# p1an-lin-jung/WavThruVec_pytorch

Measured on AMD Instinct MI355X. Metric: audio samples/sec (16 kHz) Vec2Wav generator, B=32×256-frame 768-d latents, 1/2/4/8 GPU, higher is better.
Workload: dtype f32; 1 GPU; BASELINE configs[1]: B=32/GPU x T=256 frames, 768-d latents, upsample (5,4,4,2,2) x320, ResBlock2, train-mode CondBN, f32; global_batch=32, frames=256, parallelism=single GPU

## Files before the change

### include/vec2wav_hip.h

```cpp
#ifndef VEC2WAV_HIP_H
#define VEC2WAV_HIP_H

#include <stdint.h>

#ifdef __cplusplus
extern "C" {
#endif

#define V2W_ABI_VERSION 35

#define V2W_E_ARG      (-1)
#define V2W_E_SHAPE    (-2)
#define V2W_E_ALGO     (-3)

#define V2W_ALGO_AUTO   0
#define V2W_ALGO_DIRECT 1
#define V2W_ALGO_MFMA   2
#define V2W_ALGO_BF16   4
#define V2W_ALGO_SPLIT  3
#define V2W_ALGO_WINO   5

int         v2w_abi_version(void);
const char* v2w_build_arch(void);

typedef struct { uint64_t magic; char* buf; int32_t cap; int32_t len; } v2w_name_sink;
#define V2W_NAME_SINK_MAGIC 0x5632574e414d4531ull
#define V2W_NAME_SINK_STREAM(sink) ((void*)((uintptr_t)(sink) | (uintptr_t)1))

int v2w_wn_fold_conv (const float* v, const float* g, float* wf, float* scratch,
                      int c_out, int c_in, int k, void* stream);
int v2w_wn_fold_convt(const float* v, const float* g, float* wf, float* scratch,
                      int c_in, int c_out, int k, void* stream);

int v2w_wf_transpose_flip(const float* wf, float* out, int k, int c_in, int c_out, void* stream);
int v2w_wf_gather_transpose(const float* wf, float* out, int k, int c_in, int c_out, int t_start, int t_step, int n, void* stream);

int v2w_pack_mfma(const float* wf, float* wp, int k, int c_in, int c_out, int u, void* stream);
int v2w_pack_mfma_dgrad(const float* wf, float* wp, int k, int c_in, int c_out, void* stream);
int v2w_pack_mfma_batch(const float* wf, float* wp, int k, int c_in, int c_out, int u, int n, void* stream);
int v2w_pack_wino(const float* wf, float* wpw, int k, int c_in, int c_out, void* stream);
int v2w_wino_terms(int k);

typedef struct {
    const float* v; const float* g; float* wp; float* scale;
    int32_t c_in, c_out, k, u, transposed;
    int32_t mf, ck;
    int32_t _pad;
    float* wf;
    float* wpd;
    float* wpw;
} v2w_fold_desc;
int v2w_fold_plan(v2w_fold_desc* descs, int n, int32_t* starts);
int v2w_fold_pack_batch(const v2w_fold_desc* descs_dev, const int32_t* starts_dev, int n,
                        int nblk_scale, int nblk_pack, int lds_bytes, void* stream);

typedef struct {
    const float* in;   const float* in_a;  const float* in_s;
    const float* wf;
    const float* wp;
    const float* bias;
    const float* res;  const float* res_a; const float* res_s;
    const float* add0; const float* add1;
    const float* mask_src; const float* mask_a; const float* mask_s;
    float*       out;
    int32_t B, C_in, C_out, L, k, dil;
    float   slope;
    int32_t accumulate;
    float   out_div;
    int32_t algo;
    float   mask_slope;
    int32_t in_stride, in_phase;
    int32_t pad_left;
    const void*  wps;
    const float* winv;
    int32_t in_ct, out_ct;
    float   out_slope;
    int32_t io_bf16;
    float*  rowsum_part;
    float*  splitk_ws;
    int64_t splitk_ws_bytes;
// ... 365 lines not shown
```

### wavthruvec_pytorch_amd/_hip.py

```python
from __future__ import annotations

import ctypes as C
import os
import threading

from . import build as _build

ABI_VERSION = 35
V2W_MAX_STAGES = 8
V2W_BN_SPLITS = 64
ALGO_AUTO, ALGO_DIRECT, ALGO_MFMA, ALGO_SPLIT, ALGO_BF16, ALGO_WINO = 0, 1, 2, 3, 4, 5

_fp = C.c_void_p


class Conv1dArgs(C.Structure):
    _fields_ = [('in_', _fp), ('in_a', _fp), ('in_s', _fp), ('wf', _fp), ('wp', _fp), ('bias', _fp),
                ('res', _fp), ('res_a', _fp), ('res_s', _fp), ('add0', _fp), ('add1', _fp),
                ('mask_src', _fp), ('mask_a', _fp), ('mask_s', _fp), ('out', _fp),
                ('B', C.c_int32), ('C_in', C.c_int32), ('C_out', C.c_int32), ('L', C.c_int32),
                ('k', C.c_int32), ('dil', C.c_int32), ('slope', C.c_float), ('accumulate', C.c_int32),
                ('out_div', C.c_float), ('algo', C.c_int32), ('mask_slope', C.c_float),
                ('in_stride', C.c_int32), ('in_phase', C.c_int32), ('pad_left', C.c_int32),
                ('wps', _fp), ('winv', _fp), ('in_ct', C.c_int32), ('out_ct', C.c_int32), ('out_slope', C.c_float),
                ('io_bf16', C.c_int32), ('rowsum_part', _fp), ('splitk_ws', _fp), ('splitk_ws_bytes', C.c_int64)]


class ConvT1dArgs(C.Structure):
    _fields_ = [('in_', _fp), ('wf', _fp), ('wp', _fp), ('bias', _fp), ('out', _fp), ('stats_part', _fp),
                ('B', C.c_int32), ('C_in', C.c_int32), ('C_out', C.c_int32), ('L', C.c_int32),
                ('k', C.c_int32), ('u', C.c_int32), ('slope', C.c_float), ('algo', C.c_int32), ('io_bf16', C.c_int32), ('_pad', C.c_int32),
                ('splitk_ws', _fp), ('splitk_ws_bytes', C.c_int64)]


class PairArgs(C.Structure):
    _fields_ = [('in_', _fp), ('in_a', _fp), ('in_s', _fp), ('wp1', _fp), ('bias1', _fp), ('wp2', _fp), ('bias2', _fp),
                ('add0', _fp), ('add1', _fp), ('out', _fp),
                ('B', C.c_int32), ('C', C.c_int32), ('L', C.c_int32), ('k', C.c_int32), ('dil1', C.c_int32), ('dil2', C.c_int32),
                ('res_mode', C.c_int32), ('slope', C.c_float), ('out_div', C.c_float)]


class StageArgs(C.Structure):
    _fields_ = [('in_', _fp), ('in_a', _fp), ('in_s', _fp),
                ('wp1', _fp * 4), ('bias1', _fp * 4), ('wp2', _fp * 4), ('bias2', _fp * 4),
                ('k', C.c_int32 * 4), ('dil1', C.c_int32 * 4), ('dil2', C.c_int32 * 4),
                ('out', _fp), ('nk', C.c_int32), ('B', C.c_int32), ('C', C.c_int32), ('L', C.c_int32),
                ('slope', C.c_float), ('out_div', C.c_float),
                ('post_w', _fp), ('post_b', _fp), ('post_out', _fp), ('post_k', C.c_int32), ('post_slope', C.c_float),
                ('bwd_mask1', _fp * 4), ('bwd_mid', _fp * 4), ('bwd_mask2', _fp), ('bwd_mask2_a', _fp), ('bwd_mask2_s', _fp),
                ('bwd_slope', C.c_float), ('bwd_rowsum', _fp * 4)]


class FoldDesc(C.Structure):
    _fields_ = [('v', _fp), ('g', _fp), ('wp', _fp), ('scale', _fp),
                ('c_in', C.c_int32), ('c_out', C.c_int32), ('k', C.c_int32), ('u', C.c_int32), ('transposed', C.c_int32),
                ('mf', C.c_int32), ('ck', C.c_int32), ('_pad', C.c_int32), ('wf', _fp), ('wpd', _fp), ('wpw', _fp)]


_P4 = _fp * 4
_I4 = C.c_int32 * 4


class StageSplitArgs(C.Structure):
    _fields_ = [('in_', _fp), ('in_a', _fp), ('in_s', _fp),
                ('wps1', _P4), ('sc1', _P4), ('bias1', _P4), ('wps2', _P4), ('sc2', _P4), ('bias2', _P4),
                ('k', _I4), ('dil1', _I4), ('dil2', _I4), ('out', _fp),
                ('nk', C.c_int32), ('B', C.c_int32), ('C', C.c_int32), ('L', C.c_int32),
                ('slope', C.c_float), ('out_div', C.c_float), ('bf16', C.c_int32), ('io_bf16', C.c_int32),
                ('post_w', _fp), ('post_b', _fp), ('post_out', _fp), ('post_k', C.c_int32), ('post_slope', C.c_float),
                ('up_wps', _fp), ('up_bias', _fp), ('up_out', _fp), ('up_stats_part', _fp),
                ('up_k', C.c_int32), ('up_u', C.c_int32), ('up_slope', C.c_float), ('rb1', C.c_int32),
                ('in_b', _P4), ('out_b', _P4), ('add0', _fp), ('add1', _fp)]


class BranchConvsArgs(C.Structure):
    _fields_ = [('in_', _fp * 3), ('in_a', _fp), ('in_s', _fp), ('wps', _fp * 3), ('bias', _fp * 3), ('out', _fp * 3),
                ('k', C.c_int32 * 3), ('dil', C.c_int32 * 3),
                ('nbr', C.c_int32), ('mode', C.c_int32), ('B', C.c_int32), ('C', C.c_int32), ('L', C.c_int32),
                ('slope', C.c_float), ('out_div', C.c_float), ('_pad', C.c_int32)]


class SplitDesc(C.Structure):
    _fields_ = [('v', _fp), ('g', _fp), ('wps', _fp), ('sc', _fp), ('rowscale', _fp),
                ('c_in', C.c_int32), ('c_out', C.c_int32), ('k', C.c_int32), ('mode', C.c_int32)]


_PA = _fp * V2W_MAX_STAGES


# ... 332 lines not shown
```

### wavthruvec_pytorch_amd/csrc/v2w_conv_mfma.hip

```cpp
#include <type_traits>
#include "v2w_tile.h"
#include "v2w_internal.h"
#include "v2w_wino.h"

#ifdef V2W_TIMELINE
V2W_TL_SETTER(v2w_timeline_set_tile)
#endif

namespace {

template <int MF, int U, int MI, int NI, int WM, int WN, int CK, int NPF, int RING, int EPI, bool VEC>
__global__ void __launch_bounds__(64 * WM * WN, (U == 1 && MI * NI >= 4) ? 3 : 1)
conv_tile_kernel(const MultiArgs m) {
    constexpr bool LEN = EPI == 3;
    typedef Frag<MF> F;
    typedef typename F::acc_t acc_t;
    constexpr int NTHREADS = 64 * WM * WN;
    constexpr int MT = MF * MI * WM;
    constexpr int NT = MF * NI * WN;
    constexpr int KSTEP = F::KSTEP;
    constexpr int CKG = 4 * KSTEP;
    constexpr int GPC = CK / CKG;
    constexpr int RS = TileGeom<MF, CK>::RS;
    static_assert(CK % CKG == 0, "chunk must hold whole A fragments");
    static_assert(RING == 2 || (RING == 4 && GPC == 4), "the 4-deep ring walks exactly one tap per revolution");

    extern __shared__ __attribute__((aligned(16))) float smem[];

    int pq = 0;
#pragma unroll
    for (int i = 1; i < V2W_MAX_MULTI; ++i) pq += (int)blockIdx.x >= m.start[i] ? 1 : 0;
    const TileArgs& p = m.p[pq];
    const int mtiles = p.Cout / MT;
// ... 665 lines not shown
                const int t0 = (r + pad) % U, nt = (K - t0 + U - 1) / U;
                if (left < nt) { t = t0 + left * U; break; }
                left -= nt;
            }
        }
        const int c = ch * CK + gg * CKG + j * KSTEP + lane / MF;
        const int co = mb * MF + lane % MF;
        wp[o] = tflip ? wf[((size_t)(K - 1 - t) * Cout + co) * Cin + c] : wf[((size_t)t * Cin + c) * Cout + co];
    }
}


__device__ __forceinline__ int find_layer(const int32_t* __restrict__ starts, int n, int blk) {
    int lo = 0, hi = n;
    while (hi - lo > 1) { const int mid = (lo + hi) >> 1; if (starts[mid] <= blk) lo = mid; else hi = mid; }
    return lo;
}

__global__ void __launch_bounds__(256)
fold_scale_batch_kernel(const v2w_fold_desc* __restrict__ descs, const int32_t* __restrict__ starts, int n) {
    __shared__ double red[16];
    const int li = find_layer(starts, n, blockIdx.x);
    const v2w_fold_desc d = descs[li];
    const int row = blockIdx.x - starts[li];
    const int inner = (d.transposed ? d.c_out : d.c_in) * d.k;
    const float* src = d.v + (size_t)row * inner;
    double acc = 0.0;
    if (d.g)
        for (int i = threadIdx.x; i < inner; i += 256) { const double x = (double)src[i]; acc += x * x; }
    const double n2 = v2w_block_sum(acc, red);
    if (threadIdx.x == 0) d.scale[row] = d.g ? (float)((double)d.g[row] / sqrt(n2)) : 1.f;
}

__global__ void __launch_bounds__(256)
fold_pack_batch_kernel(const v2w_fold_desc* __restrict__ descs, const int32_t* __restrict__ starts, int n) {
    extern __shared__ float tile[];
    const int li = find_layer(starts, n, blockIdx.x);
    const v2w_fold_desc d = descs[li];
    const int blk = blockIdx.x - starts[li];
    const int MF = d.mf, CK = d.ck, K = d.k, U = d.u;
    const int KSTEP = MF == 32 ? 2 : 4, CKG = 4 * KSTEP, GPC = CK / CKG, nch = d.c_in / CK;
    const int mb = blk / nch, ch = blk % nch;
    const int nrow = d.transposed ? CK : MF;
    const int rlen = (d.transposed ? MF : CK) * K;
    const int rstride = rlen + 1;
    for (int idx = threadIdx.x; idx < nrow * rlen; idx += 256) {
        const int r = idx / rlen, x = idx - r * rlen;
        const float* src = d.transposed ? d.v + ((size_t)(ch * CK + r) * d.c_out + mb * MF) * K
                                        : d.v + ((size_t)(mb * MF + r) * d.c_in + ch * CK) * K;
        const float sc = d.scale[d.transposed ? ch * CK + r : mb * MF + r];
        tile[r * rstride + x] = src[x] * sc;
    }
    __syncthreads();
    const int pad = (K - U) / 2;
    float* dst = d.wp + (size_t)(mb * nch + ch) * K * GPC * 256;
    for (int o = threadIdx.x; o < K * GPC * 256; o += 256) {
        const int j = o & 3, lane = (o >> 2) & 63;
        const int rest = o >> 8;
        const int gg = rest % GPC, ts = rest / GPC;
        int t = ts;
        if (U > 1) {
            int left = ts;
            for (int r = 0; r < U; ++r) {
                const int t0 = (r + pad) % U, nt = (K - t0 + U - 1) / U;
                if (left < nt) { t = t0 + left * U; break; }
                left -= nt;
            }
        }
        const int c = gg * CKG + j * KSTEP + lane / MF, co = lane % MF;
        dst[o] = d.transposed ? tile[c * rstride + co * K + t] : tile[co * rstride + c * K + t];
    }
    if (d.wpw && d.transposed) {
        constexpr int NT = wino_seg_terms(2), WGPC = 4;
        const int nchw = nch / 2;
        for (int o = threadIdx.x; o < U * GPC * NT * 256; o += 256) {
            const int j = o & 3, lane = (o >> 2) & 63;
            int rest = o >> 8;
            const int term = rest % NT; rest /= NT;
            const int g2 = rest % GPC, r = rest / GPC;
            const int row = r * 32 + lane % 32, co = row / U, ph = row - co * U;
            const int c = g2 * CKG + j * KSTEP + lane / MF;
            const float* w = tile + c * rstride + co * K;
            const int fi = ((ch & 1) * GPC + g2) * NT + term;
            d.wpw[((((size_t)(mb * U + r) * nchw + ch / 2) * (NT * WGPC) + fi) * 64 + lane) * 4 + j] = wino_weight(2, term, w[ph + U], w[ph], 0.f);
        }
    } else if (d.wpw) {
        const int nfr = wino_terms(K) * GPC;
        float* dw = d.wpw + (size_t)(mb * nch + ch) * nfr * 256;
        for (int o = threadIdx.x; o < nfr * 256; o += 256) {
            const int j = o & 3, lane = (o >> 2) & 63;
            int s0, ntap, gg, term;
            wino_frag(K, GPC, o >> 8, s0, ntap, gg, term);
            const int c = gg * CKG + j * KSTEP + lane / MF, co = lane % MF;
            const float* w = tile + co * rstride + c * K + s0;
            dw[o] = wino_weight(ntap, term, w[0], ntap > 1 ? w[1] : 0.f, ntap > 2 ? w[2] : 0.f);
        }
    }
    if (d.wf) {
        for (int idx = threadIdx.x; idx < K * CK * MF; idx += 256) {
            const int col = idx % MF, c = (idx / MF) % CK, t = idx / (MF * CK);
            d.wf[((size_t)t * d.c_in + ch * CK + c) * d.c_out + mb * MF + col] =
                d.transposed ? tile[c * rstride + col * K + t] : tile[col * rstride + c * K + t];
        }
    }
    if (d.wpd) {
        const int nchd = d.c_out / CK;
        float* dd = d.wpd + (size_t)(ch * nchd + mb) * K * GPC * 256;
        for (int o = threadIdx.x; o < K * GPC * 256; o += 256) {
            const int j = o & 3, lane = (o >> 2) & 63;
            const int rest = o >> 8;
            const int gg = rest % GPC, ts = rest / GPC;
            const int kc = gg * CKG + j * KSTEP + lane / MF, row = lane % MF;
            dd[o] = tile[kc * rstride + row * K + (K - 1 - ts)];
        }
    }
}

}

struct LayerCfg { int mf, ck; };
static LayerCfg v2w_layer_cfg(int c_in, int c_out, int u) {
    LayerCfg c{0, 0};
    if (c_in % 16 != 0) return c;
    if (u == 1) {
        if (c_out % 32 == 0 && c_in % 32 == 0) c = {32, 32};
        else if (c_out % 32 == 0) c = {32, 16};
        else if (c_out == 16) c = {16, 16};
    } else if (u == 2 || u == 4 || u == 5 || u == 8) {
        if (c_out % 64 == 0 || c_out == 32) c = {32, 16};
        else if (c_out == 16) c = {16, 16};
    }
    return c;
}

static int pack_mfma(const float* wf, float* wp, int k, int c_in, int c_out, int u, int n, int tflip, void* stream) {
    if (!wf || !wp || k <= 0 || c_in <= 0 || c_out <= 0 || u <= 0) return V2W_E_ARG;
    const LayerCfg cfg = v2w_layer_cfg(c_in, c_out, u);
    if (!cfg.mf) return V2W_E_SHAPE;
    const size_t total = (size_t)k * c_in * c_out;
    int grid = (int)((total + 255) / 256); if (grid > 4096) grid = 4096;
    V2W_LAUNCH(pack_mfma_kernel, dim3(grid, n), dim3(256), 0, (hipStream_t)stream, wf, wp, k, c_in, c_out, cfg.mf, cfg.ck, u, tflip);
    return v2w_launch_status();
}

extern "C" int v2w_pack_mfma(const float* wf, float* wp, int k, int c_in, int c_out, int u, void* stream) {
    return pack_mfma(wf, wp, k, c_in, c_out, u, 1, 0, stream);
}

// ... 60 lines not shown
}

int v2w_convt1d_mfma(const v2w_convt1d_args* a, hipStream_t stream, int* cfg_out, long long* ws_query, const int32_t* len, int len_mul) {
    const LayerCfg cfg = v2w_layer_cfg(a->C_in, a->C_out, a->u);
    if ((!a->wp && !cfg_out && !ws_query) || !cfg.mf) return V2W_E_SHAPE;
    TileArgs p{};
    p.cfg_out = cfg_out;
    p.splitk_ws = a->splitk_ws; p.splitk_ws_bytes = a->splitk_ws ? a->splitk_ws_bytes : 0; p.ws_query = ws_query;
    p.in = a->in; p.wp = a->wp; p.bias = a->bias; p.out = a->out; p.stats_part = a->stats_part;
    if (len && (len_mul < 1 || a->stats_part)) return V2W_E_ARG;
    p.len = len; p.len_mul = len_mul;
    p.B = a->B; p.Cin = a->C_in; p.Cout = a->C_out; p.L = a->L; p.K = a->k; p.dil = 1;
    p.CinT = p.Cin; p.CoutT = p.Cout; p.out_slope = 1.f;
    p.pad = (a->k - a->u) / 2;
    p.slope = a->slope; p.accumulate = 0; p.out_div = 0.f;
    int hl = 0, hr = 0;
    for (int r = 0; r < a->u; ++r) {
        const int rp = r + p.pad, t0 = rp % a->u, c = rp / a->u, nt = (a->k - t0 + a->u - 1) / a->u;
        if (c > hr) hr = c;
        if (nt - 1 - c > hl) hl = nt - 1 - c;
    }
    p.hl = hl; p.hr = hr;
    switch (a->u) {
        case 2: return launch_convt_u<2>(p, stream);
        case 4: return launch_convt_u<4>(p, stream);
        case 5: return launch_convt_u<5>(p, stream);
        case 8: return launch_convt_u<8>(p, stream);
        default: return V2W_E_SHAPE;
    }
}

extern "C" int v2w_fold_plan(v2w_fold_desc* descs, int n, int32_t* starts) {
    if (!descs || !starts || n <= 0) return V2W_E_ARG;
    int bs = 0, bp = 0, lds = 0;
    for (int i = 0; i < n; ++i) {
        v2w_fold_desc& d = descs[i];
        if (d.c_in <= 0 || d.c_out <= 0 || d.k <= 0 || d.u <= 0) return V2W_E_ARG;
        const LayerCfg cfg = v2w_layer_cfg(d.c_in, d.c_out, d.transposed ? d.u : 1);
        if (!cfg.mf) return V2W_E_SHAPE;
        d.mf = cfg.mf; d.ck = cfg.ck;
        if (d.wpd && (d.transposed || d.c_in != d.c_out || cfg.mf != cfg.ck)) return V2W_E_ARG;
        if (d.wpw && !d.transposed && (cfg.mf != 32 || cfg.ck != 32 || wino_terms(d.k) == 0)) return V2W_E_ARG;
        if (d.wpw && d.transposed && (cfg.mf != 32 || cfg.ck != 16 || (d.u != 2 && d.u != 4) || d.k != 2 * d.u || d.c_in % 32 != 0 || d.c_in < 64
                                      || (d.u * d.c_out) % 64 != 0)) return V2W_E_ARG;
        starts[i] = bs; starts[n + 1 + i] = bp;
        bs += d.transposed ? d.c_in : d.c_out;
        bp += (d.c_out / cfg.mf) * (d.c_in / cfg.ck);
        const int nrow = d.transposed ? cfg.ck : cfg.mf, rlen = (d.transposed ? cfg.mf : cfg.ck) * d.k;
        const int bytes = nrow * (rlen + 1) * (int)sizeof(float);
        if (bytes > lds) lds = bytes;
    }
    starts[n] = bs; starts[2 * n + 1] = bp;
    if (lds > 160 * 1024) return V2W_E_SHAPE;
    return lds;
}

extern "C" int v2w_fold_pack_batch(const v2w_fold_desc* descs_dev, const int32_t* starts_dev, int n,
                                   int nblk_scale, int nblk_pack, int lds_bytes, void* stream) {
    if (!descs_dev || !starts_dev || n <= 0 || nblk_scale <= 0 || nblk_pack <= 0 || lds_bytes <= 0) return V2W_E_ARG;
    hipStream_t st = (hipStream_t)stream;
    if (lds_bytes > 64 * 1024) {
        hipError_t e = v2w_max_lds(reinterpret_cast<const void*>(fold_pack_batch_kernel), lds_bytes, st);
        if (e != hipSuccess) return (int)e;
    }
    V2W_LAUNCH(fold_scale_batch_kernel, dim3(nblk_scale), dim3(256), 0, st, descs_dev, starts_dev, n);
    V2W_LAUNCH(fold_pack_batch_kernel, dim3(nblk_pack), dim3(256), lds_bytes, st, descs_dev, starts_dev + n + 1, n);
    return v2w_launch_status();
}
```

### wavthruvec_pytorch_amd/forward_plan.py

```python
from __future__ import annotations

import contextlib
import functools
from collections import namedtuple

import torch

from . import hipops

LRELU_SLOPE = 0.1
POST_SLOPE = 0.01
_Z_CHANNEL = 128


class DirectStreams:

    def __init__(self, main, side, side2=None):
        self.main, self.side, self.side2 = main, side, side if side2 is None else side2
        self.events = {}
        self.nfork = 1
        self.tag = None

    def stream(self, sid):
        return (self.main, self.side, self.side2)[sid]
# ... 192 lines not shown
    @functools.cached_property
    def stg(self):
        return self.g.stage_record(self.stage_i)

    def buf(self, name, shape, dtype=torch.float32):
        return self.g._buf(name, shape, dtype=dtype, device=self.dev)

    def lkw(self, mul=None):
        if self.lens is None:
            return {}
        return dict(lengths=self.lens, len_mul=self.lmul if mul is None else mul)

    def lkw_out(self):
        return self.lkw(self.lmul * self.g.ups[self.stage_i].stride)

    def wino_streams(self, kind='wpw'):
        return self.g._fold_key.get(kind, {})

    def weights(self):
        g, st, dev = self.g, self.st, self.dev
        B, ns = self.B, self.ns
        self.gbs = [self.buf(f'gb.{i}', (B, 2 * g.cbns[i].num_features)) for i in range(ns)]
        self.z_ws = self.buf('z_ws', (ns * B * _Z_CHANNEL,))
        self.sigma_ws = self.buf('sigma_ws', (ns,))
        self.affs = None
        self.cond_ran = False
        if self.cond_sid == 2:
            self.cond()
        with (self.on_side() if st else contextlib.nullcontext()):
            self.wf, self.wp = g._fold_weights(dev, need_wf=self.save is not None, bf16_only=st)
        self.wps = g._split_weights(dev, all_ups=st, ups_stream=self.S.side, mark=self.mark if st else None,
                                    between=self.cond if st else None)
        self.cond()

    def cond(self):
        if self.cond_ran:
            return
        self.cond_ran = True
        g, dev, ns, B = self.g, self.dev, self.ns, self.B
        with self.on_side(self.cond_sid):
            if not self.training and self.save is None:
                sn_p = [q for c in g.cbns for q in (c.layer.weight_orig, c.layer.weight_u, c.layer.weight_v)]
                skey = (tuple((q.data_ptr(), q._version) for q in sn_p), str(dev))
                if g._fold_key.get('sigma') != skey:
                    hipops.cond_sigma([c.layer.weight_orig.detach() for c in g.cbns], [c.layer.weight_u for c in g.cbns],
                                      [c.layer.weight_v for c in g.cbns], self.sigma_ws, training=False)
                    g._fold_key['sigma'] = skey
                self.affs = [(self.buf(f'bn.a{i}', (B, g.cbns[i].num_features)), self.buf(f'bn.s{i}', (B, g.cbns[i].num_features))) for i in range(ns)]
                hipops.cond_affine_eval(
                    self.spk, self.nz, [f.weight.detach() for f in g.fcs], [f.bias.detach() for f in g.fcs],
                    [c.layer.weight_orig.detach() for c in g.cbns], [c.layer.bias.detach() for c in g.cbns], self.sigma_ws,
                    [c.batch_nrom.running_mean for c in g.cbns], [c.batch_nrom.running_var for c in g.cbns],
                    [c.batch_nrom.eps for c in g.cbns], [q[0] for q in self.affs], [q[1] for q in self.affs])
            else:
                g._fold_key.pop('sigma', None)
                hipops.cond_gamma_beta(
                    self.spk, self.nz, [f.weight.detach() for f in g.fcs], [f.bias.detach() for f in g.fcs],
                    [c.layer.weight_orig.detach() for c in g.cbns], [c.layer.bias.detach() for c in g.cbns],
                    [c.layer.weight_u for c in g.cbns], [c.layer.weight_v for c in g.cbns], self.gbs, self.z_ws, self.sigma_ws, self.training)
        if self.st:
            self.mark('cond', self.cond_sid)

    def ck(self, nm, io=3):
        g = self.g
        if nm in self.wps32:
            return dict(algo=hipops.ALGO_BF16, wps=self.wps32[nm])
# ... 388 lines not shown
```

### wavthruvec_pytorch_amd/hipops.py

```python
from __future__ import annotations

import ctypes as C
from typing import Optional, Sequence

import torch

from . import _hip

ALGO_AUTO, ALGO_DIRECT, ALGO_MFMA, ALGO_SPLIT, ALGO_BF16, ALGO_WINO = (_hip.ALGO_AUTO, _hip.ALGO_DIRECT, _hip.ALGO_MFMA, _hip.ALGO_SPLIT,
                                                                        _hip.ALGO_BF16, _hip.ALGO_WINO)


def _chk(t: Optional[torch.Tensor], name: str, dtype=torch.float32):
    if t is None:
        return
    if not t.is_cuda:
        raise RuntimeError(f'{name} must live on a GPU: the Vec2Wav HIP path has no CPU fallback')
    if t.dtype != dtype:
        raise TypeError(f'{name} must be {dtype}, got {t.dtype}')
    if not t.is_contiguous():
        raise RuntimeError(f'{name} must be contiguous')


def _stream(t: torch.Tensor) -> int:
# ... 525 lines not shown


def convt_stats_tiles(B, c_in, c_out, L, k, u):
    cfg = (C.c_int32 * 10)()
    a = _convt_shape(B, c_in, c_out, L, k, u)
    return int(cfg[9]) if _hip.load().v2w_convt1d_tile_config(C.byref(a), cfg) == 0 else 0


def bn_reduce_partials(part, ntiles, Cc, count, stats):
    _hip.check(_hip.load().v2w_bn_reduce_partials(part.data_ptr(), ntiles, Cc, float(count), stats.data_ptr(), _stream(part)),
               'v2w_bn_reduce_partials')
    return stats


def bn_reduce_finalize(part, ntiles, count, stats, gb, running_mean, running_var, num_batches_tracked, a_out, s_out, *, momentum=0.1, eps=1e-5):
    B, C2 = gb.shape
    _hip.check(_hip.load().v2w_bn_reduce_finalize(part.data_ptr(), ntiles, float(count), gb.data_ptr(), running_mean.data_ptr(),
                                                  running_var.data_ptr(), _hip.ptr(num_batches_tracked), stats.data_ptr(), a_out.data_ptr(),
                                                  s_out.data_ptr(), B, C2 // 2, momentum, eps, _stream(gb)), 'v2w_bn_reduce_finalize')
    return a_out, s_out


class FoldPlan:

    def __init__(self, layers, device):
        n = len(layers)
        self.n = n
        layers = [tuple(l) + (None,) * (11 - len(l)) for l in layers]
        rows = [(l[3] if l[7] else l[4]) for l in layers]
        self.scale = torch.empty((sum(rows),), device=device, dtype=torch.float32)
        descs = (_hip.FoldDesc * n)()
        off = 0
        for d, (v, g, wp, ci, co, k, u, tr, wf, wpd, wpw), r in zip(descs, layers, rows):
            d.v = v.data_ptr(); d.g = _hip.ptr(g); d.wp = wp.data_ptr()
            d.wf = _hip.ptr(wf); d.wpd = _hip.ptr(wpd); d.wpw = _hip.ptr(wpw)
            d.scale = self.scale.data_ptr() + 4 * off
            d.c_in, d.c_out, d.k, d.u, d.transposed = ci, co, k, u, int(tr)
            off += r
        starts = (C.c_int32 * (2 * (n + 1)))()
        lds = _hip.load().v2w_fold_plan(descs, n, starts)
        _hip.check(0 if lds > 0 else (lds or -1), 'v2w_fold_plan')
        self.lds = lds
        self.nblk_scale, self.nblk_pack = starts[n], starts[2 * n + 1]
        self.descs_dev = torch.frombuffer(bytearray(bytes(descs)), dtype=torch.uint8).to(device)
        self.starts_dev = torch.tensor(list(starts), dtype=torch.int32, device=device)
        self.key = tuple((v.data_ptr(), 0 if g is None else g.data_ptr(), wp.data_ptr()) for (v, g, wp, *_r) in layers)

    def run(self):
        _hip.check(_hip.load().v2w_fold_pack_batch(self.descs_dev.data_ptr(), self.starts_dev.data_ptr(), self.n,
                                                   self.nblk_scale, self.nblk_pack, self.lds,
                                                   torch.cuda.current_stream(self.scale.device).cuda_stream),
                   'v2w_fold_pack_batch')


class SplitPlan:

    def __init__(self, layers, device, bf16=False):
        n = len(layers)
        self.n = n
        self.bf16 = bool(bf16)
        self.rowscale = torch.empty((sum(v.shape[0] for v, *_ in layers),), device=device, dtype=torch.float32)
        descs = (_hip.SplitDesc * n)()
        starts = [0] * (2 * (n + 1))
        off = blocks = 0
        for i, (d, (v, g, wps, sc)) in enumerate(zip(descs, layers)):
            co, ci, k = v.shape
            d.v = v.data_ptr(); d.g = _hip.ptr(g); d.wps = wps.data_ptr(); d.sc = sc.data_ptr()
            d.rowscale = self.rowscale.data_ptr() + 4 * off
            d.c_in, d.c_out, d.k, d.mode = ci, co, k, int(bf16)
            starts[i], starts[n + 1 + i] = off, blocks
            off += co
            blocks += ((co + 31) // 32) * (ci // 16)
        starts[n], starts[2 * n + 1] = off, blocks
        self.nblk_rows, self.nblk_pack = off, blocks
        self.k_max = max(v.shape[2] for v, *_ in layers)
        self.descs_dev = torch.frombuffer(bytearray(bytes(descs)), dtype=torch.uint8).to(device)
        self.starts_dev = torch.tensor(starts, dtype=torch.int32, device=device)
        self.key = tuple((v.data_ptr(), 0 if g is None else g.data_ptr(), w.data_ptr()) for (v, g, w, _s) in layers)

# ... 894 lines not shown
```

### wavthruvec_pytorch_amd/models.py

```python
from __future__ import annotations

import math
import warnings
from typing import Dict, List, Optional

import contextlib
import torch
import torch.nn as nn

from . import _hip, hipops
from .modules import ConditionalBatchNorm1d
from .utils import get_padding, init_weights

LRELU_SLOPE = 0.1
_SIDE_STREAMS: Dict[str, 'torch.cuda.Stream'] = {}
_CAPTURE_STREAMS: Dict[str, 'torch.cuda.Stream'] = {}
_Z_CHANNEL = 128


class _WNConvBase(nn.Module):
    transposed = False

    def __init__(self, in_channels, out_channels, kernel_size, stride=1, dilation=1, padding=0):
        super().__init__()
# ... 328 lines not shown
        wpw_up = {}
        for name, m in layers:
            if bf16_only and name != 'conv_post':
                wf[name], wp[name] = None, None
                continue
            v, g = (m.weight_v.detach(), m.weight_g.detach()) if m.weight_normed else (m.weight.detach(), None)
            u = m.stride if m.transposed else 1
            mfma_ok = (self.algo != hipops.ALGO_DIRECT and name != 'conv_post' and
                       hipops.conv_tile_config(1, m.in_channels, m.out_channels, 64, m.kernel_size,
                                               1 if m.transposed else m.dilation, u) is not None)
            wpwb = None
            if (mfma_ok and wino and not m.transposed and hipops.wino_terms(m.kernel_size) and m.in_channels % 32 == 0 and m.in_channels >= 64
                    and m.out_channels % 64 == 0 and (m.out_channels >= 128 or m.dilation == 1)):
                wpwb = wpw[name] = self._wbuf('wpw.' + name, (hipops.wino_terms(m.kernel_size) * m.in_channels * m.out_channels,), device=device)
            if mfma_ok and name in stage_names:
                wpwb = wpw_stage[name] = self._wbuf('wpw.' + name, (hipops.wino_terms(m.kernel_size) * m.in_channels * m.out_channels,), device=device)
            if mfma_ok and wpwb is None and name in sum_names:
                wpwb = wpw_sum[name] = self._wbuf('wpw.' + name, (hipops.wino_terms(m.kernel_size) * m.in_channels * m.out_channels,), device=device)
            if mfma_ok and name in up_names:
                wpwb = wpw_up[name] = self._wbuf('wpw.' + name, (3 * m.stride * m.out_channels * m.in_channels,), device=device)
            if mfma_ok and need_wf:
                n_el = m.kernel_size * m.in_channels * m.out_channels
                wfb = self._wbuf('wf.' + name, (m.kernel_size, m.in_channels, m.out_channels), device=device)
                wpb = self._wbuf('wp.' + name, (n_el,), device=device)
                wdb = None
                if not m.transposed and m.in_channels == m.out_channels and name.startswith('resblocks.'):
                    wdb = wpd[name] = self._wbuf('wpd.' + name, (n_el,), device=device)
                batch.append((v, g, wpb, m.in_channels, m.out_channels, m.kernel_size, u, m.transposed, wfb, wdb, wpwb))
                wf[name], wp[name] = wfb, wpb
            elif mfma_ok:
                wpb = self._wbuf('wp.' + name, (m.kernel_size * m.in_channels * m.out_channels,), device=device)
                batch.append((v, g, wpb, m.in_channels, m.out_channels, m.kernel_size, u, m.transposed, None, None, wpwb))
                wf[name], wp[name] = None, wpb
            else:
                wfb = self._wbuf('wf.' + name, (m.kernel_size, m.in_channels, m.out_channels), device=device)
                scratch = self._wbuf('wf_scratch', (max(2048, m.out_channels, m.in_channels),), device=device)
                (hipops.fold_convt_weight if m.transposed else hipops.fold_conv_weight)(v, g, wfb, scratch)
                wf[name], wp[name] = wfb, None
        if batch:
            key = tuple((q[0].data_ptr(), 0 if q[1] is None else q[1].data_ptr(), q[2].data_ptr(),
                         0 if len(q) < 9 or q[8] is None else q[8].data_ptr(), 0 if len(q) < 11 or q[10] is None else q[10].data_ptr()) for q in batch)
            plan = self._fold_key.get('plan')
            if plan is None or plan.key != key:
                self._drop_tapes()
                plan = hipops.FoldPlan(batch, device)
                plan.key = key
                self._fold_key['plan'] = plan
            plan.run()
        self._fold_key.update(state=state, wf=wf, wp=wp, wpd=wpd, wpw=wpw, wpw_stage=wpw_stage, wpw_sum=wpw_sum, wpw_up=wpw_up, vers=tuple(vers), gen=self._fold_key.get('gen', 0) + 1)
        return wf, wp

    def stage_record(self, i):
        from .forward_plan import Stage
        js = range(i * self.num_kernels, (i + 1) * self.num_kernels)
        return Stage(i, self.ups[i].out_channels, tuple(self.resblocks[j] for j in js), tuple(f'resblocks.{j}' for j in js))

    def _rb2_stage_layers(self, selected, cs):
        stages = (self.stage_record(i) for i in range(self.num_upsamples))
        return {nm for stg in stages if stg.is_rb2 and selected(stg) for nm in stg.layers(cs)}

    def _wino_stage_layers(self):
        from .forward_plan import stage_wino_selected
        return self._rb2_stage_layers(lambda stg: stage_wino_selected(self.wino_stage, self.precision, self.algo, stg.C, stg.blocks), (0, 1))

    def _wino_up_layers(self):
        from .forward_plan import wino_up_selected
        return {f'ups.{i}' for i, up in enumerate(self.ups)
                if wino_up_selected(self.wino_up, i, self.precision, self.algo, up.in_channels, up.out_channels, up.kernel_size, up.stride)}

    def _wino_sum_layers(self):
        from .forward_plan import wino_sum_selected
        return self._rb2_stage_layers(lambda stg: wino_sum_selected(self.wino_sum, self.precision, self.algo, stg.C, stg.pairs(1)), (1,))

# ... 256 lines not shown
```

Before: 364.0 million samples/s.

## Restructure batched weight-norm fold/pack kernel with vectorized stores and cost-sorted scheduling

Rewrites the batched fold+pack kernel. Tile loads are now row-wise and optionally float4-vectorized, the tap map and Winograd fragment tables are precomputed in LDS, and packed slots are written as 4-wide stores. The host plan orders pack blocks by estimated cost, largest first, and adds a 'plain' descriptor mode so non-MFMA layers are folded inside the same batched launch instead of through separate per-layer fold calls. The forward plan also joins the side stream early for large training batches. These changes add shape checks and more code paths in exchange for fewer launches and better-coalesced weight-preparation traffic.

```diff
diff --git a/include/vec2wav_hip.h b/include/vec2wav_hip.h
--- a/include/vec2wav_hip.h
+++ b/include/vec2wav_hip.h
@@ -45,7 +45,7 @@
     const float* v; const float* g; float* wp; float* scale;
     int32_t c_in, c_out, k, u, transposed;
     int32_t mf, ck;
-    int32_t _pad;
+    int32_t flags;
     float* wf;
     float* wpd;
     float* wpw;
diff --git a/wavthruvec_pytorch_amd/_hip.py b/wavthruvec_pytorch_amd/_hip.py
--- a/wavthruvec_pytorch_amd/_hip.py
+++ b/wavthruvec_pytorch_amd/_hip.py
@@ -54,7 +54,7 @@
 class FoldDesc(C.Structure):
     _fields_ = [('v', _fp), ('g', _fp), ('wp', _fp), ('scale', _fp),
                 ('c_in', C.c_int32), ('c_out', C.c_int32), ('k', C.c_int32), ('u', C.c_int32), ('transposed', C.c_int32),
-                ('mf', C.c_int32), ('ck', C.c_int32), ('_pad', C.c_int32), ('wf', _fp), ('wpd', _fp), ('wpw', _fp)]
+                ('mf', C.c_int32), ('ck', C.c_int32), ('flags', C.c_int32), ('wf', _fp), ('wpd', _fp), ('wpw', _fp)]
 
 
 _P4 = _fp * 4
diff --git a/wavthruvec_pytorch_amd/csrc/v2w_conv_mfma.hip b/wavthruvec_pytorch_amd/csrc/v2w_conv_mfma.hip
--- a/wavthruvec_pytorch_amd/csrc/v2w_conv_mfma.hip
+++ b/wavthruvec_pytorch_amd/csrc/v2w_conv_mfma.hip
@@ -1,4 +1,6 @@
+#include <algorithm>
 #include <type_traits>
+#include <vector>
 #include "v2w_tile.h"
 #include "v2w_internal.h"
 #include "v2w_wino.h"
@@ -730,88 +732,155 @@
     if (threadIdx.x == 0) d.scale[row] = d.g ? (float)((double)d.g[row] / sqrt(n2)) : 1.f;
 }
 
+__device__ __forceinline__ int find_pack_layer(const int32_t* __restrict__ starts, int n, int blk) {
+    int li = 0, best = -1;
+    for (int i = 0; i < n; ++i) { const int s = starts[i]; if (s <= blk && s > best) { best = s; li = i; } }
+    return li;
+}
+
+constexpr int FOLD_VEC = 1;
+constexpr int FOLD_MAX_TAPS = 160;
+constexpr int FOLD_MAX_FRAGS = 256;
+
+typedef float __attribute__((address_space(1))) gfloat;
+typedef float gfloat4v __attribute__((ext_vector_type(4)));
+typedef gfloat4v __attribute__((address_space(1))) gfloat4;
+template <bool VEC>
+__device__ __forceinline__ void fold_store_slot(gfloat* __restrict__ dst, float a, float b, float c, float e) {
+    if (VEC) *(gfloat4*)dst = gfloat4v{a, b, c, e};
+    else { dst[0] = a; dst[1] = b; dst[2] = c; dst[3] = e; }
+}
+
+__device__ __forceinline__ void fold_plain_block(const v2w_fold_desc& dd, int blk) {
+    struct { const gfloat* v; const gfloat* scale; gfloat* wf; int k, c_in, c_out, transposed; } d =
+        {(const gfloat*)dd.v, (const gfloat*)dd.scale, (gfloat*)dd.wf, dd.k, dd.c_in, dd.c_out, dd.transposed};
+    const int total = d.k * d.c_in * d.c_out;
+    const int end = min(total, (blk + 1) * 1024);
+    for (int idx = blk * 1024 + (int)threadIdx.x; idx < end; idx += 256) {
+        const int o = idx % d.c_out, rest = idx / d.c_out, c = rest % d.c_in, t = rest / d.c_in;
+        d.wf[idx] = d.transposed ? d.v[((size_t)c * d.c_out + o) * d.k + t] * d.scale[c] : d.v[((size_t)o * d.c_in + c) * d.k + t] * d.scale[o];
+    }
+}
+
+template <bool VEC>
+__device__ __forceinline__ void fold_pack_block(const v2w_fold_desc& dd, int blk, float* __restrict__ tile, int* __restrict__ tapmap,
+                                                int* __restrict__ fragtab) {
+    struct { const gfloat* v; const gfloat* scale; gfloat* wp; gfloat* wf; gfloat* wpd; gfloat* wpw; int c_in, c_out, k, u, transposed, mf, ck; } d =
+        {(const gfloat*)dd.v, (const gfloat*)dd.scale, (gfloat*)dd.wp, (gfloat*)dd.wf, (gfloat*)dd.wpd, (gfloat*)dd.wpw,
+         dd.c_in, dd.c_out, dd.k, dd.u, dd.transposed, dd.mf, dd.ck};
+    const int tid = threadIdx.x;
+    const int MF = d.mf, CK = d.ck, K = d.k, U = d.u;
+    const bool tr = d.transposed != 0;
+    const int mshift = MF == 32 ? 5 : 4;
+    const int KSTEP = MF == 32 ? 2 : 4, CKG = 4 * KSTEP, GPC = CK / CKG, gshift = GPC == 4 ? 2 : (GPC == 2 ? 1 : 0), nch = d.c_in / CK;
+    const int mb = blk / nch, ch = blk - mb * nch;
+    const int nrow = tr ? CK : MF;
+    const int rlen = (tr ? MF : CK) * K;
+    const int rstride = rlen + 1;
+    {
+        const int sub = tid & 31;
+        for (int r = tid >> 5; r < nrow; r += 8) {
+            const gfloat* src = tr ? d.v + ((size_t)(ch * CK + r) * d.c_out + mb * MF) * K
+                                  : d.v + ((size_t)(mb * MF + r) * d.c_in + ch * CK) * K;
+            const float sc = d.scale[tr ? ch * CK + r : mb * MF + r];
+            float* row = tile + r * rstride;
+            if (VEC) {
+                for (int x = 4 * sub; x < rlen; x += 128) {
+                    const gfloat4v q = *(const gfloat4*)(src + x);
+                    row[x] = q.x * sc; row[x + 1] = q.y * sc; row[x + 2] = q.z * sc; row[x + 3] = q.w * sc;
+                }
+            } else {
+                for (int x = sub; x < rlen; x += 32) row[x] = src[x] * sc;
+            }
+        }
+    }
+    if (tr && tid < K) {
+        const int pad = (K - U) / 2;
+        int t = tid, left = tid;
+        for (int r = 0; r < U; ++r) {
+            const int t0 = (r + pad) % U, nt = (K - t0 + U - 1) / U;
+            if (left < nt) { t = t0 + left * U; break; }
+            left -= nt;
+        }
+        tapmap[tid] = t;
+    }
+    const int nfr = (d.wpw && !tr) ? wino_terms(K) * GPC : 0;
+    if (tid < nfr) {
+        int s0, ntap, gg, term;
+        wino_frag(K, GPC, tid, s0, ntap, gg, term);
+        fragtab[tid] = s0 | (ntap << 8) | (gg << 12) | (term << 16);
+    }
+    __syncthreads();
+    const int lane = tid & 63, lk = lane >> mshift, co = lane & (MF - 1);
+    const int cstep = tr ? rstride : K, ostep = tr ? K : rstride;
+    if (d.wp) {
+        gfloat* dst = d.wp + (size_t)(mb * nch + ch) * K * GPC * 256;
+        for (int s = tid; s < K * GPC * 64; s += 256) {
+            const int f = s >> 6, gg = f & (GPC - 1), ts = f >> gshift;
+            const int t = tr ? tapmap[ts] : ts;
+            const float* w = tile + co * ostep + (gg * CKG + lk) * cstep + t;
+            fold_store_slot<VEC>(dst + 4 * s, w[0], w[KSTEP * cstep], w[2 * KSTEP * cstep], w[3 * KSTEP * cstep]);
+        }
+    }
+    if (d.wpw && tr) {
+        constexpr int NT = wino_seg_terms(2), WGPC = 4;
+        const int nchw = nch / 2, ushift = U == 4 ? 2 : 1;
+        for (int s = tid; s < U * GPC * NT * 64; s += 256) {
+            int rest = s >> 6;
+            const int term = rest % NT; rest /= NT;
+            const int g2 = rest & (GPC - 1), r = rest >> gshift;
+            const int row = r * 32 + (lane & 31), oc = row >> ushift, ph = row & (U - 1);
+            const float* w = tile + (g2 * CKG + lk) * rstride + oc * K;
+            const int fi = ((ch & 1) * GPC + g2) * NT + term;
+            gfloat* dst = d.wpw + ((((size_t)(mb * U + r) * nchw + ch / 2) * (NT * WGPC) + fi) * 64 + lane) * 4;
+            const int js = KSTEP * rstride;
+            fold_store_slot<VEC>(dst, wino_weight(2, term, w[ph + U], w[ph], 0.f), wino_weight(2, term, w[js + ph + U], w[js + ph], 0.f),
+                                 wino_weight(2, term, w[2 * js + ph + U], w[2 * js + ph], 0.f),
+                                 wino_weight(2, term, w[3 * js + ph + U], w[3 * js + ph], 0.f));
+        }
+    } else if (d.wpw) {
+        gfloat* dw = d.wpw + (size_t)(mb * nch + ch) * nfr * 256;
+        const int js = KSTEP * K;
+        for (int s = tid; s < nfr * 64; s += 256) {
+            const int e = fragtab[s >> 6], s0 = e & 255, ntap = (e >> 8) & 15, gg = (e >> 12) & 15, term = e >> 16;
+            const float* w = tile + co * rstride + (gg * CKG + lk) * K + s0;
+            float q[4];
+#pragma unroll
+            for (int j = 0; j < 4; ++j)
+                q[j] = wino_weight(ntap, term, w[j * js], ntap > 1 ? w[j * js + 1] : 0.f, ntap > 2 ? w[j * js + 2] : 0.f);
+            fold_store_slot<VEC>(dw + 4 * s, q[0], q[1], q[2], q[3]);
+        }
+    }
+    if (d.wf) {
+        const int cshift = CK == 32 ? 5 : 4;
+        for (int i4 = tid; i4 < (K * CK * MF) >> 2; i4 += 256) {
+            const int idx = 4 * i4, col = idx & (MF - 1), c = (idx >> mshift) & (CK - 1), t = idx >> (mshift + cshift);
+            const float* w = tile + col * ostep + c * cstep + t;
+            fold_store_slot<VEC>(d.wf + ((size_t)t * d.c_in + ch * CK + c) * d.c_out + mb * MF + col, w[0], w[ostep], w[2 * ostep], w[3 * ostep]);
+        }
+    }
+    if (d.wpd) {
+        const int nchd = d.c_out / CK;
+        gfloat* dg = d.wpd + (size_t)(ch * nchd + mb) * K * GPC * 256;
+        for (int s = tid; s < K * GPC * 64; s += 256) {
+            const int f = s >> 6, gg = f & (GPC - 1), ts = f >> gshift;
+            const float* w = tile + (gg * CKG + lk) * rstride + co * K + (K - 1 - ts);
+            fold_store_slot<VEC>(dg + 4 * s, w[0], w[KSTEP * rstride], w[2 * KSTEP * rstride], w[3 * KSTEP * rstride]);
+        }
+    }
+}
+
 __global__ void __launch_bounds__(256)
 fold_pack_batch_kernel(const v2w_fold_desc* __restrict__ descs, const int32_t* __restrict__ starts, int n) {
     extern __shared__ float tile[];
-    const int li = find_layer(starts, n, blockIdx.x);
+    __shared__ int tapmap[FOLD_MAX_TAPS];
+    __shared__ int fragtab[FOLD_MAX_FRAGS];
+    const int li = find_pack_layer(starts, n, blockIdx.x);
     const v2w_fold_desc d = descs[li];
     const int blk = blockIdx.x - starts[li];
-    const int MF = d.mf, CK = d.ck, K = d.k, U = d.u;
-    const int KSTEP = MF == 32 ? 2 : 4, CKG = 4 * KSTEP, GPC = CK / CKG, nch = d.c_in / CK;
-    const int mb = blk / nch, ch = blk % nch;
-    const int nrow = d.transposed ? CK : MF;
-    const int rlen = (d.transposed ? MF : CK) * K;
-    const int rstride = rlen + 1;
-    for (int idx = threadIdx.x; idx < nrow * rlen; idx += 256) {
-        const int r = idx / rlen, x = idx - r * rlen;
-        const float* src = d.transposed ? d.v + ((size_t)(ch * CK + r) * d.c_out + mb * MF) * K
-                                        : d.v + ((size_t)(mb * MF + r) * d.c_in + ch * CK) * K;
-        const float sc = d.scale[d.transposed ? ch * CK + r : mb * MF + r];
-        tile[r * rstride + x] = src[x] * sc;
-    }
-    __syncthreads();
-    const int pad = (K - U) / 2;
-    float* dst = d.wp + (size_t)(mb * nch + ch) * K * GPC * 256;
-    for (int o = threadIdx.x; o < K * GPC * 256; o += 256) {
-        const int j = o & 3, lane = (o >> 2) & 63;
-        const int rest = o >> 8;
-        const int gg = rest % GPC, ts = rest / GPC;
-        int t = ts;
-        if (U > 1) {
-            int left = ts;
-            for (int r = 0; r < U; ++r) {
-                const int t0 = (r + pad) % U, nt = (K - t0 + U - 1) / U;
-                if (left < nt) { t = t0 + left * U; break; }
-                left -= nt;
-            }
-        }
-        const int c = gg * CKG + j * KSTEP + lane / MF, co = lane % MF;
-        dst[o] = d.transposed ? tile[c * rstride + co * K + t] : tile[co * rstride + c * K + t];
-    }
-    if (d.wpw && d.transposed) {
-        constexpr int NT = wino_seg_terms(2), WGPC = 4;
-        const int nchw = nch / 2;
-        for (int o = threadIdx.x; o < U * GPC * NT * 256; o += 256) {
-            const int j = o & 3, lane = (o >> 2) & 63;
-            int rest = o >> 8;
-            const int term = rest % NT; rest /= NT;
-            const int g2 = rest % GPC, r = rest / GPC;
-            const int row = r * 32 + lane % 32, co = row / U, ph = row - co * U;
-            const int c = g2 * CKG + j * KSTEP + lane / MF;
-            const float* w = tile + c * rstride + co * K;
-            const int fi = ((ch & 1) * GPC + g2) * NT + term;
-            d.wpw[((((size_t)(mb * U + r) * nchw + ch / 2) * (NT * WGPC) + fi) * 64 + lane) * 4 + j] = wino_weight(2, term, w[ph + U], w[ph], 0.f);
-        }
-    } else if (d.wpw) {
-        const int nfr = wino_terms(K) * GPC;
-        float* dw = d.wpw + (size_t)(mb * nch + ch) * nfr * 256;
-        for (int o = threadIdx.x; o < nfr * 256; o += 256) {
-            const int j = o & 3, lane = (o >> 2) & 63;
-            int s0, ntap, gg, term;
-            wino_frag(K, GPC, o >> 8, s0, ntap, gg, term);
-            const int c = gg * CKG + j * KSTEP + lane / MF, co = lane % MF;
-            const float* w = tile + co * rstride + c * K + s0;
-            dw[o] = wino_weight(ntap, term, w[0], ntap > 1 ? w[1] : 0.f, ntap > 2 ? w[2] : 0.f);
-        }
-    }
-    if (d.wf) {
-        for (int idx = threadIdx.x; idx < K * CK * MF; idx += 256) {
-            const int col = idx % MF, c = (idx / MF) % CK, t = idx / (MF * CK);
-            d.wf[((size_t)t * d.c_in + ch * CK + c) * d.c_out + mb * MF + col] =
-                d.transposed ? tile[c * rstride + col * K + t] : tile[col * rstride + c * K + t];
-        }
-    }
-    if (d.wpd) {
-        const int nchd = d.c_out / CK;
-        float* dd = d.wpd + (size_t)(ch * nchd + mb) * K * GPC * 256;
-        for (int o = threadIdx.x; o < K * GPC * 256; o += 256) {
-            const int j = o & 3, lane = (o >> 2) & 63;
-            const int rest = o >> 8;
-            const int gg = rest % GPC, ts = rest / GPC;
-            const int kc = gg * CKG + j * KSTEP + lane / MF, row = lane % MF;
-            dd[o] = tile[kc * rstride + row * K + (K - 1 - ts)];
-        }
-    }
+    if (d.mf == 0) fold_plain_block(d, blk);
+    else if (d.flags & FOLD_VEC) fold_pack_block<true>(d, blk, tile, tapmap, fragtab);
+    else fold_pack_block<false>(d, blk, tile, tapmap, fragtab);
 }
 
 }
@@ -938,27 +1007,50 @@
 
 extern "C" int v2w_fold_plan(v2w_fold_desc* descs, int n, int32_t* starts) {
     if (!descs || !starts || n <= 0) return V2W_E_ARG;
-    int bs = 0, bp = 0, lds = 0;
+    int bs = 0, lds = 0;
+    std::vector<int> nblk(n), order(n);
+    std::vector<long long> cost(n);
     for (int i = 0; i < n; ++i) {
         v2w_fold_desc& d = descs[i];
-        if (d.c_in <= 0 || d.c_out <= 0 || d.k <= 0 || d.u <= 0) return V2W_E_ARG;
+        if (d.c_in <= 0 || d.c_out <= 0 || d.k <= 0 || d.u <= 0 || !d.v || !d.scale) return V2W_E_ARG;
+        const long long total = (long long)d.k * d.c_in * d.c_out;
+        if (total > 0x7fffffffll - 1024) return V2W_E_SHAPE;
         const LayerCfg cfg = v2w_layer_cfg(d.c_in, d.c_out, d.transposed ? d.u : 1);
-        if (!cfg.mf) return V2W_E_SHAPE;
+        order[i] = i;
+        starts[i] = bs;
+        bs += d.transposed ? d.c_in : d.c_out;
+        d.flags = 0;
+        const bool plain = !d.wp && !d.wpd && !d.wpw && d.wf;
+        if (!cfg.mf && !plain) return V2W_E_SHAPE;
+        if (plain) {
+            d.mf = d.ck = 0;
+            nblk[i] = (int)((total + 1023) / 1024);
+            cost[i] = 1024;
+            continue;
+        }
         d.mf = cfg.mf; d.ck = cfg.ck;
+        if (!d.wp && !d.wpw) return V2W_E_ARG;
+        if (d.transposed && d.k > FOLD_MAX_TAPS) return V2W_E_SHAPE;
         if (d.wpd && (d.transposed || d.c_in != d.c_out || cfg.mf != cfg.ck)) return V2W_E_ARG;
         if (d.wpw && !d.transposed && (cfg.mf != 32 || cfg.ck != 32 || wino_terms(d.k) == 0)) return V2W_E_ARG;
         if (d.wpw && d.transposed && (cfg.mf != 32 || cfg.ck != 16 || (d.u != 2 && d.u != 4) || d.k != 2 * d.u || d.c_in % 32 != 0 || d.c_in < 64
                                       || (d.u * d.c_out) % 64 != 0)) return V2W_E_ARG;
-        starts[i] = bs; starts[n + 1 + i] = bp;
-        bs += d.transposed ? d.c_in : d.c_out;
-        bp += (d.c_out / cfg.mf) * (d.c_in / cfg.ck);
-        const int nrow = d.transposed ? cfg.ck : cfg.mf, rlen = (d.transposed ? cfg.mf : cfg.ck) * d.k;
-        const int bytes = nrow * (rlen + 1) * (int)sizeof(float);
-        if (bytes > lds) lds = bytes;
-    }
-    starts[n] = bs; starts[2 * n + 1] = bp;
-    if (lds > 160 * 1024) return V2W_E_SHAPE;
-    return lds;
+        if (d.wpw && !d.transposed && wino_terms(d.k) * 4 > FOLD_MAX_FRAGS) return V2W_E_SHAPE;
+        if (v2w_al16(d.v) && v2w_al16(d.wp) && v2w_al16(d.wf) && v2w_al16(d.wpd) && v2w_al16(d.wpw)) d.flags |= FOLD_VEC;
+        nblk[i] = (d.c_out / cfg.mf) * (d.c_in / cfg.ck);
+        const int nstream = (d.wp ? 1 : 0) + (d.wf ? 1 : 0) + (d.wpd ? 1 : 0);
+        cost[i] = (long long)cfg.mf * cfg.ck * (d.k * (1 + nstream) + (!d.wpw ? 0 : d.transposed ? 3 * d.u : wino_terms(d.k)));
+        const long long rlen = (long long)(d.transposed ? cfg.mf : cfg.ck) * d.k;
+        const long long bytes = (d.transposed ? cfg.ck : cfg.mf) * (rlen + 1) * (long long)sizeof(float);
+        if (bytes > 160 * 1024) return V2W_E_SHAPE;
+        if ((int)bytes > lds) lds = (int)bytes;
+    }
+    std::stable_sort(order.begin(), order.end(), [&](int a, int b) { return cost[a] > cost[b]; });
+    long long bp = 0;
+    for (int j = 0; j < n; ++j) { starts[n + 1 + order[j]] = (int32_t)bp; bp += nblk[order[j]]; }
+    if (bp > 0x7fffffffll) return V2W_E_SHAPE;
+    starts[n] = bs; starts[2 * n + 1] = (int32_t)bp;
+    return lds > 16 ? lds : 16;
 }
 
 extern "C" int v2w_fold_pack_batch(const v2w_fold_desc* descs_dev, const int32_t* starts_dev, int n,
diff --git a/wavthruvec_pytorch_amd/forward_plan.py b/wavthruvec_pytorch_amd/forward_plan.py
--- a/wavthruvec_pytorch_amd/forward_plan.py
+++ b/wavthruvec_pytorch_amd/forward_plan.py
@@ -248,6 +248,8 @@
         self.wps = g._split_weights(dev, all_ups=st, ups_stream=self.S.side, mark=self.mark if st else None,
                                     between=self.cond if st else None)
         self.cond()
+        if not st and self.training and self.B * self.T >= 3072:
+            self.join_side()
 
     def cond(self):
         if self.cond_ran:
diff --git a/wavthruvec_pytorch_amd/hipops.py b/wavthruvec_pytorch_amd/hipops.py
--- a/wavthruvec_pytorch_amd/hipops.py
+++ b/wavthruvec_pytorch_amd/hipops.py
@@ -581,7 +581,7 @@
         descs = (_hip.FoldDesc * n)()
         off = 0
         for d, (v, g, wp, ci, co, k, u, tr, wf, wpd, wpw), r in zip(descs, layers, rows):
-            d.v = v.data_ptr(); d.g = _hip.ptr(g); d.wp = wp.data_ptr()
+            d.v = v.data_ptr(); d.g = _hip.ptr(g); d.wp = _hip.ptr(wp)
             d.wf = _hip.ptr(wf); d.wpd = _hip.ptr(wpd); d.wpw = _hip.ptr(wpw)
             d.scale = self.scale.data_ptr() + 4 * off
             d.c_in, d.c_out, d.k, d.u, d.transposed = ci, co, k, u, int(tr)
@@ -593,7 +593,7 @@
         self.nblk_scale, self.nblk_pack = starts[n], starts[2 * n + 1]
         self.descs_dev = torch.frombuffer(bytearray(bytes(descs)), dtype=torch.uint8).to(device)
         self.starts_dev = torch.tensor(list(starts), dtype=torch.int32, device=device)
-        self.key = tuple((v.data_ptr(), 0 if g is None else g.data_ptr(), wp.data_ptr()) for (v, g, wp, *_r) in layers)
+        self.key = tuple((v.data_ptr(), 0 if g is None else g.data_ptr(), 0 if wp is None else wp.data_ptr()) for (v, g, wp, *_r) in layers)
 
     def run(self):
         _hip.check(_hip.load().v2w_fold_pack_batch(self.descs_dev.data_ptr(), self.starts_dev.data_ptr(), self.n,
diff --git a/wavthruvec_pytorch_amd/models.py b/wavthruvec_pytorch_amd/models.py
--- a/wavthruvec_pytorch_amd/models.py
+++ b/wavthruvec_pytorch_amd/models.py
@@ -384,13 +384,17 @@
                 wpb = self._wbuf('wp.' + name, (m.kernel_size * m.in_channels * m.out_channels,), device=device)
                 batch.append((v, g, wpb, m.in_channels, m.out_channels, m.kernel_size, u, m.transposed, None, None, wpwb))
                 wf[name], wp[name] = None, wpb
+            elif self.algo != hipops.ALGO_DIRECT and not bf16_only:
+                wfb = self._wbuf('wf.' + name, (m.kernel_size, m.in_channels, m.out_channels), device=device)
+                batch.append((v, g, None, m.in_channels, m.out_channels, m.kernel_size, u, m.transposed, wfb, None, None))
+                wf[name], wp[name] = wfb, None
             else:
                 wfb = self._wbuf('wf.' + name, (m.kernel_size, m.in_channels, m.out_channels), device=device)
                 scratch = self._wbuf('wf_scratch', (max(2048, m.out_channels, m.in_channels),), device=device)
                 (hipops.fold_convt_weight if m.transposed else hipops.fold_conv_weight)(v, g, wfb, scratch)
                 wf[name], wp[name] = wfb, None
         if batch:
-            key = tuple((q[0].data_ptr(), 0 if q[1] is None else q[1].data_ptr(), q[2].data_ptr(),
+            key = tuple((q[0].data_ptr(), 0 if q[1] is None else q[1].data_ptr(), 0 if q[2] is None else q[2].data_ptr(),
                          0 if len(q) < 9 or q[8] is None else q[8].data_ptr(), 0 if len(q) < 11 or q[10] is None else q[10].data_ptr()) for q in batch)
             plan = self._fold_key.get('plan')
             if plan is None or plan.key != key:
```

New measurement: 364.3 million samples/s (median of 6 runs). No clear change (+0.1%).
